# snap-research/3dgp

Measured on AMD Instinct MI355X. Metric: generator-forward img/s @256^2, 64 steps, higher is better.
Workload: dtype f32; 1 GPU; BASELINE configs[2]: ImageNet 256x256, 64(+64) ray steps, cmax 512, c_dim 1000, tri-plane 512^2 x 96, full HIP path; batch_per_gpu=16, global_batch=16, img_resolution=256, num_ray_steps=64, depth_adaptor=False, parallelism=dp1 (batch-sharded, weights replicated)

## Files before the change

### 3dgp_amd/_lib.py

```python
import ctypes
import os
from ctypes import POINTER, c_char_p, c_double, c_float, c_int, c_int32, c_int64, c_void_p

import torch

_HERE = os.path.dirname(os.path.abspath(__file__))
LIB_PATH = os.path.join(_HERE, 'csrc', 'libtdgp_hip.so')

P = c_void_p
_PROTOTYPES = {
    'tdgp_version': (c_int, []),
    'tdgp_last_error': (c_char_p, []),
    'tdgp_profile_enable': (c_int, [c_int]),
    'tdgp_profile_report': (c_int64, [c_char_p, c_int64]),
    'tdgp_device_fault': (c_int, [c_int]),
    'tdgp_bias_act': (c_int, [P, P, P, c_int64, c_int, c_int64, c_int, c_float, c_float, c_float, c_int, P]),
    'tdgp_bias_act_grad': (c_int, [P, P, P, P, P, P, c_int64, c_int, c_int64, c_int, c_int, c_float, c_float, c_float, c_int, P]),
    'tdgp_upfirdn2d': (c_int, [P, P, P, c_int, c_int, c_int, c_int, POINTER(c_int64), c_int, c_int, POINTER(c_int64),
                               c_int, c_int, c_int, c_int, c_int, c_int, c_int, c_int, c_int, c_int, c_int, c_float, c_int, P]),
    'tdgp_modconv_pack_bytes': (c_int64, [c_int, c_int, c_int]),
    'tdgp_modconv_pack': (c_int, [P, P, c_int, c_int, c_int, P]),
    'tdgp_modconv2d_workspace_bytes': (c_int64, [c_int, c_int, c_int, c_int, c_int, c_int, c_int]),
    'tdgp_modconv2d_takes_folded_up2': (c_int, [c_int, c_int, c_int, c_int, c_int]),
    'tdgp_modconv2d_path': (c_int, [c_int, c_int, c_int, c_int, c_int, c_int, c_int, c_int, c_int]),
    'tdgp_conv2d': (c_int, [P, P, P, P, c_int, c_int, c_int, c_int, c_int, c_int, c_int, c_int, c_int, c_int, P]),
    'tdgp_conv2d_weight_grad_workspace_bytes': (c_int64, [c_int, c_int, c_int, c_int, c_int]),
    'tdgp_conv2d_weight_grad': (c_int, [P, P, P, P, c_int64, c_int, c_int, c_int, c_int, c_int, c_int, c_int, c_int, c_int, c_int, P]),
    'tdgp_conv_transpose2d_x2': (c_int, [P, P, P, P, c_int, c_int, c_int, c_int, c_int, P, c_int64, P]),
    'tdgp_set_conv_arith': (c_int, [c_int]),
    'tdgp_modconv_wsq_offset': (c_int64, [c_int, c_int, c_int]),
    'tdgp_demod_batch': (c_int, [P, P, P, c_int, c_int, c_int, P]),
    'tdgp_modconv2d': (c_int, [P, P, P, P, P, c_int64, P, POINTER(c_float), P, P, c_int, c_int, c_int, c_int, c_int, c_int, c_int,
                               c_int, c_int, c_float, c_float, c_float, c_int, c_int, P, c_int64, P]),
    'tdgp_modconv2d_bf16': (c_int, [P, P, P, P, P, c_int64, P, POINTER(c_float), P, P, c_int, c_int, c_int, c_int, c_int, c_int, c_int,
                                    c_int, c_int, c_float, c_float, c_float, c_int, c_int, P, c_int64, P]),
    'tdgp_cast_f32_bf16': (c_int, [P, P, c_int64, P]),
    'tdgp_style_affine': (c_int, [P, P, P, P, P, P, c_int, c_int, c_int, c_int, P]),
    'tdgp_cam2world': (c_int, [P, P, P, P, c_int, P]),
    'tdgp_sample_rays': (c_int, [P, P, c_int, P, P, P, P, c_int, c_int, c_int, P]),
    'tdgp_sample_stratified': (c_int, [P, P, P, c_int64, c_int, c_int, c_float, c_float, P]),
    'tdgp_density_activation': (c_int, [P, P, c_int64, c_int, c_float, P]),
    'tdgp_planes_to_hwc': (c_int, [P, P, c_int, c_int, c_int, c_int, P]),
    'tdgp_triplane_features': (c_int, [P, P, P, c_int, c_int64, c_int, c_int, c_int, c_float, P]),
    'tdgp_triplane_field': (c_int, [P, P, P, P, P, P, P, P, P, P, c_float, P, P, c_int, c_int64, c_int, c_int, c_int, c_int, c_int, c_int, c_float,
                                    c_int, P]),
    'tdgp_ray_march': (c_int, [P, P, P, P, P, P, P, c_int64, c_int, c_int, c_int, c_int, c_float, c_float, P]),
    'tdgp_triplane_field_grad_workspace_bytes': (c_int64, [c_int, c_int64, c_int, c_int]),
    'tdgp_triplane_field_grad': (c_int, [P, P, P, P, P, P, P, P, P, P, P, P, P, P, c_int64, c_int, c_int64, c_int, c_int, c_int, c_int, c_float, c_int, P]),
    'tdgp_triplane_field_deep': (c_int, [P, P, P, P, P, P, P, c_int, P, c_float, P, P, c_int, c_int64, c_int, c_int, c_int, c_int, c_int, c_int, c_float,
                                         c_int, P]),
    'tdgp_triplane_field_deep_grad_workspace_bytes': (c_int64, [c_int, c_int64, c_int, c_int, c_int]),
    'tdgp_triplane_field_deep_grad': (c_int, [P, P, P, P, c_int, P, P, P, P, P, P, c_int64, c_int, c_int64, c_int, c_int, c_int, c_int, c_float, c_int, P]),
    'tdgp_ray_march_grad': (c_int, [P, P, P, P, P, P, P, P, c_int64, c_int, c_int, c_int, c_int, c_float, P]),
    'tdgp_sample_importance': (c_int, [P, P, P, P, P, P, P, P, c_int64, c_int, c_int, c_int, c_int, P]),
    'tdgp_unify_samples': (c_int, [P, P, P, c_int, P, P, P, c_int, P, P, P, P, c_int64, c_int, P]),
    'tdgp_importance_from_coarse': (c_int, [P, P, P, P, P, P, P, c_int64, c_int, c_int, c_int, c_int, c_float, c_float, c_float, c_float, P]),
    'tdgp_merge_composite': (c_int, [P, P, c_int, P, P, c_int, P, P, P, P, P, P, c_int64, c_int, c_int, c_float, c_float, P]),
    'tdgp_render_fused_workspace_bytes': (c_int64, [c_int, c_int64, c_int, c_int]),
    'tdgp_render_fused': (c_int, [P] * 13 + [c_int, c_int64, c_int, c_int, c_int, c_int, c_int, c_int, c_int, c_float, c_float, c_float, c_int, c_int, c_float, P, c_int64, P]),
    'tdgp_rays_to_image': (c_int, [P, P, c_int, c_int, P]),
    'tdgp_frames_to_grid_u8': (c_int, [P, c_int64, c_int, c_int, c_int, P, c_int, c_int, c_int64, c_int64, c_int, c_int, c_int, c_float, c_float, P]),
    'tdgp_ppl_frames': (c_int, [P, c_int64, c_int, c_int, c_int, c_int, c_int, P, P]),
    'tdgp_pair_sqdist_workspace_bytes': (c_int64, [c_int64, c_int64]),
    'tdgp_pair_sqdist': (c_int, [P, c_int64, c_int64, c_double, P, P, c_int64, P]),
    'tdgp_voxel_coords': (c_int, [P, c_int64, c_int64, c_int, c_float, c_float, c_float, c_float, P]),
    'tdgp_mcubes_workspace_bytes': (c_int64, [c_int, c_int, c_int]),
    'tdgp_mcubes_count': (c_int, [P, c_int, c_int, c_int, c_float, P, c_int64, P]),
    'tdgp_mcubes_emit': (c_int, [P, c_int, c_int, c_int, c_float, P, c_int64, P, c_int64, P, c_int64, P]),
    'tdgp_iso_bracket': (c_int, [P, c_int64, P, c_int64, c_int, c_int, c_float, P, P, P]),
    'tdgp_iso_locate': (c_int, [P, c_int64, P, P, P, c_int64, P, P, P, c_int64, c_int, c_int, c_float, c_float, c_float, P, P, P, P]),
    'tdgp_iso_shade': (c_int, [P, P, P, c_int64, c_int, POINTER(c_float), c_float, POINTER(c_float), POINTER(c_float), P, P, P]),
    'tdgp_mesh_visibility': (c_int, [P, c_int64, P, c_int64, P, P, P, c_int, c_int, c_int, c_float, c_int, P, P]),
    'tdgp_mesh_resolve': (c_int, [P, P, c_int64, P, c_int64, P, P, c_int64, c_float, c_float, P, P, P, P, P, P, P, P]),
    'tdgp_mesh_shade': (c_int, [P, P, P, P, c_int64, c_int, POINTER(c_float), c_float, POINTER(c_float), POINTER(c_float), P, P]),
    'tdgp_mesh_visibility_ms': (c_int, [P, c_int64, P, c_int64, P, P, c_int, c_int, c_int, c_int, c_float, c_int, P, P]),
    'tdgp_mesh_resolve_ms': (c_int, [P, P, c_int64, P, c_int64, P, P, c_int, c_int, c_int, c_int, c_float, P, P, P, c_int, c_int, c_int, c_int, c_int, c_int,
                                     POINTER(c_float), c_float, POINTER(c_float), POINTER(c_float), P, P, P, P, P, P, P]),
    'tdgp_mesh_labels_workspace_bytes': (c_int64, [c_int64, c_int64]),
    'tdgp_mesh_labels': (c_int, [P, c_int64, c_int64, P, P, c_int64, P]),
    'tdgp_mesh_component_ids_workspace_bytes': (c_int64, [c_int64]),
    'tdgp_mesh_component_ids': (c_int, [P, c_int64, P, P, c_int64, P]),
    'tdgp_mesh_component_stats': (c_int, [P, P, c_int64, c_int64, P, c_int64, P, P, P, P, P, P, P, P]),
# ... 108 lines not shown

def byte_workspace(query_name, dims, device, refusal, at_least=0):
    need = int(getattr(load(), query_name)(*dims))
    if need < 0:
        raise refusal
    return torch.empty([max(need, at_least)], dtype=torch.uint8, device=device), need


def require_cuda(t, what):
    if not (isinstance(t, torch.Tensor) and t.is_cuda):
        raise RuntimeError(f'{what} must reside on the GPU (got {getattr(t, "device", type(t))}); the HIP ops have no CPU path')


def f32c(t):
    if t.dtype != torch.float32:
        t = t.float()
    return t.contiguous()


def profile_enable(on=True):
    load().tdgp_profile_enable(int(bool(on)))


def profile_report():
    lib = load()
    need = lib.tdgp_profile_report(None, 0)
    buf = ctypes.create_string_buffer(int(need) + 16)
    lib.tdgp_profile_report(buf, len(buf))
    out = {}
    for line in buf.value.decode().splitlines():
        name, n, tot, mn, mx = line.split()
        out[name] = dict(launches=int(n), total_ms=float(tot), avg_ms=float(tot) / max(int(n), 1), min_ms=float(mn), max_ms=float(mx))
    return out


def device_fault(clear=False):
    return int(load().tdgp_device_fault(int(bool(clear))))


def raise_on_device_fault(where=''):
    code = device_fault(clear=True)
    if code:
        raise RuntimeError(f'libtdgp_hip: device fault {code} reported{" in " + where if where else ""}: a bounded in-kernel wait ran out, '
                           'the results of that launch are invalid (the fault word has been cleared)')


def set_conv_arith(mode):
    lib = load()
    prev = int(lib.tdgp_set_conv_arith(int(mode)))
    if prev < 0:
        msg = lib.tdgp_last_error()
        raise RuntimeError(f'tdgp_set_conv_arith failed ({prev}): {msg.decode() if msg else "?"}')
    return prev
```

### 3dgp_amd/build.py

```python
import os
import subprocess
import sys
from concurrent.futures import ThreadPoolExecutor

HERE = os.path.dirname(os.path.abspath(__file__))
CSRC = os.path.join(HERE, 'csrc')
LIB = os.path.join(CSRC, 'libtdgp_hip.so')
SOURCES = ['core.hip', 'bias_act.hip', 'upfirdn2d.hip', 'modconv.hip', 'conv_grad.hip', 'camera_rays.hip', 'frames_grid.hip', 'field.hip', 'field_deep.hip', 'sampling.hip', 'render_grad.hip', 'render_fused.hip', 'geometry.hip', 'iso_surface.hip', 'mesh_raster.hip', 'mesh_components.hip', 'mesh_surface.hip', 'mesh_simplify.hip', 'mesh_texture.hip', 'metrics.hip', 'pair_dist.hip', 'gaussian.hip', 'augment.hip', 'step_tail.hip', 'resample.hip']
HEADERS = ['common.h', 'device_scan.h', 'shade.h', 'mesh_bary.h', 'mesh_hit.h', 'modconv_bf16.inc', 'modconv_wino.inc', 'modconv_wino4.inc', 'modconv_wino4f.inc', 'modconv_host.inc', 'field_body.inc', 'field_grad.inc', 'field_walk2.inc', 'mc_table.inc', os.path.join('..', '..', 'include', 'tdgp.h')]
FLAGS = ['--offload-arch=gfx950', '-O3', '-std=c++17', '-ffp-contract=off', '-fPIC', '-fvisibility=hidden',
         '-Wno-unused-result']


def _hipcc():
    for c in (os.environ.get('HIPCC'), '/opt/rocm/bin/hipcc', 'hipcc'):
        if c and (os.path.isabs(c) and os.path.exists(c) or not os.path.isabs(c)):
            return c
    raise RuntimeError('hipcc not found')


def _stale(target, deps):
    if not os.path.exists(target):
        return True
    t = os.path.getmtime(target)
    return any(os.path.getmtime(d) > t for d in deps)


def _isa_check_module():
    sys.path.insert(0, HERE)
    try:
        import isa_check
    finally:
        sys.path.pop(0)
    return isa_check


def _verify_isa(asm_path, what, check_name):
    isa_check = _isa_check_module()
    skip = os.environ.get('TDGP_SKIP_ISA_CHECK', '0') not in ('', '0')
    try:
        res = getattr(isa_check, check_name)(open(asm_path).read())
        bad = [(k, why, ins) for k, (_, v) in res.items() for why, ins in v]
        msg = None
        if not res:
            msg = f'no {what} instantiation found in the listing'
        elif bad:
            msg = '; '.join(f'{k}: {why} | {ins}' for k, why, ins in bad[:8])
    except isa_check.IsaListingError as e:
        res, msg = {}, f'listing not understood: {e}'
    if msg:
        full = f'ISA check of {what} failed (3dgp_amd/isa_check.py): {msg}'
        if skip:
            import warnings
            warnings.warn(full + ' -- TDGP_SKIP_ISA_CHECK is set: continuing')
            return res
        os.remove(asm_path)
        raise RuntimeError(full + ' (TDGP_SKIP_ISA_CHECK=1 downgrades this to a warning)')
    return res


def verify_field_isa(asm_path):
    return _verify_isa(asm_path, 'triplane_walk2_kernel', 'check_walk2_asm')


def verify_modconv_isa(asm_path):
    res = dict(_verify_isa(asm_path, 'conv3_wino4_kernel', 'check_wino4_asm'))
    res.update(_verify_isa(asm_path, 'conv3_wino4f_kernel', 'check_wino4f_asm'))
    res.update(_verify_isa(asm_path, 'torgb_mfma_kernel (FAST)', 'check_torgb_asm'))
    return res


def build_native(force=False, verbose=False):
    hipcc = _hipcc()
    objdir = os.path.join(CSRC, 'build')
    os.makedirs(objdir, exist_ok=True)
    hdrs = [os.path.join(CSRC, h) for h in HEADERS]
    jobs = []
    for src in SOURCES:
        s = os.path.join(CSRC, src)
        o = os.path.join(objdir, src.replace('.hip', '.o'))
        if force or _stale(o, [s] + hdrs):
            jobs.append((s, o))

    def compile_one(job):
        s, o = job
        cmd = [hipcc] + FLAGS + ['-c', s, '-o', o]
        if verbose:
            print(' '.join(cmd), file=sys.stderr)
        r = subprocess.run(cmd, capture_output=True, text=True)
        if r.returncode != 0:
            raise RuntimeError(f'hipcc failed for {s}:\n{r.stderr}')
        return o

    checked = [('field.hip', 'field.s', verify_field_isa), ('modconv.hip', 'modconv.s', verify_modconv_isa)]
    todo = []
    for src, lst, fn in checked:
        sp, ap = os.path.join(CSRC, src), os.path.join(objdir, lst)
        if any(s == sp for s, _ in jobs) or _stale(ap, [sp] + hdrs):
            todo.append((sp, ap, fn))

    def asm_one(item):
        sp, ap, _ = item
        r = subprocess.run([hipcc] + FLAGS + ['-S', '--cuda-device-only', '-o', ap, sp], capture_output=True, text=True)
        if r.returncode != 0:
            raise RuntimeError(f'hipcc -S failed for {sp}:\n{r.stderr}')

    with ThreadPoolExecutor(max_workers=min(8, max(1, len(jobs) + len(todo)))) as ex:
        futs = [ex.submit(asm_one, it) for it in todo]
        list(ex.map(compile_one, jobs))
        for f in futs:
            f.result()
    for _, ap, fn in todo:
        fn(ap)
    objs = [os.path.join(objdir, s.replace('.hip', '.o')) for s in SOURCES]
    if force or jobs or _stale(LIB, objs):
        cmd = [hipcc, '--offload-arch=gfx950', '-shared', '-fPIC', '-o', LIB] + objs
        r = subprocess.run(cmd, capture_output=True, text=True)
        if r.returncode != 0:
            raise RuntimeError(f'link failed:\n{r.stderr}')
    return LIB


if __name__ == '__main__':
    print(build_native(force='--force' in sys.argv, verbose=True))
```

### 3dgp_amd/csrc/modconv.hip

```cpp
#include <type_traits>
#include "common.h"
#include <stdlib.h>

#define TDGP_WAVE_INDEX(tid) __builtin_amdgcn_readfirstlane((tid) >> 6)

namespace {

typedef float f32x16 __attribute__((ext_vector_type(16)));

constexpr int KC3 = 4;

struct TapTable {
    int ntaps, halo;
    int tap_w[25];
    int tap_off_y[25];
    int tap_off_x[25];
    int gridH, gridW;
};

struct EpiParams {
    const float* __restrict__ dcoef; const float* __restrict__ noise; const float* __restrict__ bias; const float* __restrict__ skip;
    float* __restrict__ y;
    int64_t noise_bstride;
    float fir[16];
// ... 2076 lines not shown
                    float v = acc[o] * d;
                    if (YBF) v = fir_round_bf16(v);
                    if (p.noise && ox0 + lx + o < p.OW) {
                        const float nq[4] = {nzv[hrow].x, nzv[hrow].y, nzv[hrow].z, nzv[hrow].w};
                        v = v + (nz_vec ? nq[o] : p.noise[b * p.noise_bstride + (int64_t)oy * p.OW + ox0 + lx + o]);
                        if (YBF) v = fir_round_bf16(v);
                    }
                    v = v + bv;
                    if constexpr (LRELU) {
                        v = __builtin_fmaxf(v, v * p.alpha) * p.gain;
                        if (p.clamp >= 0.f) v = __builtin_amdgcn_fmed3f(v, -p.clamp, p.clamp);
                    }
                    else {
                        v = act_apply(v, p.act, p.alpha) * p.gain;
                        if (p.clamp >= 0.f) v = v < -p.clamp ? -p.clamp : (v > p.clamp ? p.clamp : v);
                    }
                    out[o] = v;
                }
                if constexpr (YBF) {
                    uint16_t* yp = p.y16 + yoff;
                    if (ox0 + lx + 3 < p.OW && (p.OW & 3) == 0) *(uint2*)yp = make_uint2(fir_pack_bf16(out[0], out[1]), fir_pack_bf16(out[2], out[3]));
                    else
                        for (int o = 0; o < 4 && ox0 + lx + o < p.OW; o++) yp[o] = (uint16_t)(fir_pack_bf16(out[o], 0.f) & 0xffffu);
                } else {
                    float* yp = p.y + yoff;
                    if (ox0 + lx + 3 < p.OW && (p.OW & 3) == 0) *(float4*)yp = make_float4(out[0], out[1], out[2], out[3]);
                    else
                        for (int o = 0; o < 4 && ox0 + lx + o < p.OW; o++) yp[o] = out[o];
                }
            }
        }
    }
}

__global__ __launch_bounds__(256) void z_gather_kernel(const float* __restrict__ z, float* __restrict__ y, int64_t rows, int OHt, int OWt, int P2, int GS2,
                                                       int ksplit, int64_t zslice) {
    for (int64_t r = blockIdx.x; r < rows; r += gridDim.x) {
        const int i = (int)(r % OHt);
        const int64_t bc = r / OHt;
        const float* zp = z + bc * 2 * GS2 + (i & 1) * GS2 + (int64_t)(i >> 1) * P2;
        float* yp = y + r * OWt;
        for (int j = threadIdx.x; j < OWt; j += blockDim.x) {
            float v = zp[j];
            for (int k = 1; k < ksplit; k++) v += zp[k * zslice + j];
            yp[j] = v;
        }
    }
}

#include "modconv_bf16.inc"
#include "modconv_wino.inc"
#include "modconv_wino4.inc"
#include "modconv_wino4f.inc"

__global__ __launch_bounds__(1024) void demod_kernel(const float* __restrict__ styles, const float* __restrict__ wsq, float* __restrict__ d, int B,
                                                    int Cin, int Cout, int CoutP) {
    __shared__ float red[16][64];
    const int ol = threadIdx.x & 63, cs = threadIdx.x >> 6;
    const int o = blockIdx.x * 64 + ol, b = blockIdx.y;
    float acc = 0.f;
    if (o < Cout)
        for (int c = cs; c < Cin; c += 16) {
            const float s = styles[b * Cin + c];
            acc = fmaf_(s * s, wsq[(int64_t)c * CoutP + o], acc);
        }
    red[cs][ol] = acc;
    __syncthreads();
    if (cs == 0 && o < Cout) {
        float t = 0.f;
#pragma unroll
        for (int k = 0; k < 16; k++) t += red[k][ol];
        d[b * Cout + o] = 1.0f / sqrtf(t + 1e-8f);
    }
}

__global__ __launch_bounds__(1024) void demod_batch_kernel(const float* __restrict__ styles_all, const int64_t* __restrict__ meta, float* __restrict__ dcoef_all, int B) {
    __shared__ float red[16][64];
    const int64_t* m = meta + (int64_t)blockIdx.z * 6;
    const float* wsq = (const float*)m[0];
    const int Cin = (int)m[2], Cout = (int)m[3], CoutP = (int)m[4];
    const float* styles = styles_all + m[1];
    float* d = dcoef_all + m[5];
    const int ol = threadIdx.x & 63, cs = threadIdx.x >> 6;
    const int o = blockIdx.x * 64 + ol, b = blockIdx.y;
    if (blockIdx.x * 64 >= Cout) return;
    float acc = 0.f;
    if (o < Cout)
        for (int c = cs; c < Cin; c += 16) {
            const float s = styles[b * Cin + c];
            acc = fmaf_(s * s, wsq[(int64_t)c * CoutP + o], acc);
        }
    red[cs][ol] = acc;
    __syncthreads();
    if (cs == 0 && o < Cout) {
        float t = 0.f;
#pragma unroll
        for (int k = 0; k < 16; k++) t += red[k][ol];
        d[b * Cout + o] = 1.0f / sqrtf(t + 1e-8f);
    }
}

__global__ __launch_bounds__(256) void pack_kernel(const float* __restrict__ w, float* __restrict__ wp, float* __restrict__ wsq, int Cout, int Cin, int T,
                                                  int KC, int CoutP, int nchunks) {
    const int64_t total = (int64_t)nchunks * T * KC * CoutP;
    for (int64_t i = blockIdx.x * (int64_t)blockDim.x + threadIdx.x; i < total; i += (int64_t)gridDim.x * blockDim.x) {
        const int c8 = (int)(i % KC);
// ... 37 lines not shown
```

### 3dgp_amd/csrc/modconv_host.inc

```

constexpr int W4_VCAP_MB = 4095;
constexpr int W4_VSMALL_MB = 192;
constexpr int W4_VSMALL_MINB = 2;
constexpr int WINO_MIN_CIN = 64;

namespace {

inline int round_up(int a, int b) { return (a + b - 1) / b * b; }

struct PackInfo {
    int T, KC, CoutP, nchunks, niter16, nch32, nch8, nch4, nsl64;
    int64_t wp_floats, wsq_floats, wsplit_floats, wbf_floats, wino_floats, wino4_floats;
    int64_t wp, wsq, wsplit, wbf, wino, wino4, total;
};
inline PackInfo pack_info(int Cout, int Cin, int k) {
    PackInfo pi;
    pi.T = k * k;
    pi.KC = KC3;
    pi.CoutP = round_up(Cout, 4);
    pi.nchunks = round_up((Cin + pi.KC - 1) / pi.KC, k == 1 ? 16 : 2);
    pi.wp_floats = (int64_t)pi.nchunks * pi.T * pi.KC * pi.CoutP;
    pi.wsq_floats = (int64_t)Cin * pi.CoutP;
    pi.niter16 = (Cin + 15) / 16;
    pi.wsplit_floats = k == 3 ? (int64_t)pi.niter16 * 9 * 3 * pi.CoutP * 8 : 0;
// ... 41 lines not shown
    p.ksplit = ks;
    p.partial = partial;
    dim3 grid(gx, gy, ks);
    TDGP_LAUNCH("conv_mfma_kernel", (conv_mfma_kernel<MTW, NTW, WM, WN, KCS, MAXT>), grid, dim3(256), lds, s, p);
    if (ks > 1)
        TDGP_LAUNCH("splitk_reduce_kernel", splitk_reduce_kernel, dim3((int)min((int64_t)2048, cdiv64(slice, 256))), dim3(256), 0, s, partial, ks, p.e);
    return 0;
}

inline int tail_ksplit(int blocks, int niter, double flop, int64_t slice_floats, int max_ks) {
    double best = 1e30;
    int ks = 1;
    for (int k = 1; k <= max_ks && k <= 4 && niter / k >= 16; k++) {
        const int n = blocks * k, full = n / 512, rem = n % 512;
        const double rounds = full + (rem == 0 ? 0.0 : (rem <= 256 ? 0.7 : 1.0));
        const double t = rounds * (flop / n) / (100e12 / 512) * 1e6 + (k - 1) * (double)slice_floats * 4.0 / 4e12 * 1e6;
        if (t < best * 0.97) { best = t; ks = k; }
    }
    return ks;
}

struct UpPlan { int cfg, BM, BN, G1, GS, ksplit; int64_t zslice; };
inline UpPlan up_plan(int B, int Cin, int Cout, int H, int W) {
    UpPlan u;
    u.cfg = Cout > 64 ? 0 : 1;
    u.BM = Cout > 64 ? 128 : 64; u.BN = Cout > 64 ? 64 : 128;
    u.G1 = W + 2;
    u.GS = round_up((H + 1) * (W + 2), 32);
    u.zslice = (int64_t)B * Cout * 4 * u.GS;
    const int blocks = cdiv(B * u.GS, u.BN) * cdiv(Cout, u.BM);
    const int niter = cdiv(Cin, 4);
    int ks;
    if (blocks < 256) {
        ks = pick_ksplit(blocks, niter);
        const int64_t cap = ((int64_t)64 << 20) / 4;
        while (ks > 1 && ks * u.zslice > cap) ks--;
    } else {
        ks = tail_ksplit(blocks, niter, 2.0 * Cin * Cout * 9.0 * H * W * B, u.zslice, 4);
    }
    u.ksplit = ks;
    return u;
}

template <int MTW, int NTW, int WM, int WN, bool DEEP>
void launch_upconv(const UpParams& u, hipStream_t s) {
    constexpr int BM = 32 * MTW * WM, BN = 32 * NTW * WN, NW = WM * WN;
    constexpr int stage = 2 * (9 * BM * 4 + 2 * (BN + 2) * 4), epi = NW * 32 * UP_CT_W;
    const size_t lds = (size_t)(stage > epi ? stage : epi) * sizeof(float);
    TDGP_ONCE_PER_DEVICE((void)hipFuncSetAttribute((const void*)upconv_mfma_kernel<MTW, NTW, WM, WN, DEEP>, hipFuncAttributeMaxDynamicSharedMemorySize, (int)lds););
    dim3 grid(cdiv(u.B * u.GS, BN), cdiv(u.Cout, BM), u.ksplit);
    TDGP_LAUNCH("upconv_mfma_kernel", (upconv_mfma_kernel<MTW, NTW, WM, WN, DEEP>), grid, dim3(64 * NW), lds, s, u);
}

template <int MT, bool RESIDENT, bool FAST, bool XBF>
void launch_torgb_v(const RgbParams& r, hipStream_t s) {
    constexpr int BM = 32 * MT;
    const size_t lds = (size_t)(16 * BM * 4 + 16 * 128 * 4 + BM) * sizeof(float);
    TDGP_ONCE_PER_DEVICE((void)hipFuncSetAttribute((const void*)torgb_mfma_kernel<MT, RESIDENT, FAST, XBF>, hipFuncAttributeMaxDynamicSharedMemorySize, (int)lds););
    RgbParams rr = r;
    const int64_t ntiles = cdiv64(r.P, 128);
    if constexpr (RESIDENT && FAST && !XBF) {
        const int cus = tdgp_cu_count();
        if (r.e.skip && ntiles >= (int64_t)cus * 8) {
            constexpr size_t lds_ws = (size_t)(16 * BM * 4 + 2 * 16 * 128 * 4 + 4 * MT * 32 * CT_LD + BM) * sizeof(float);
            TDGP_ONCE_PER_DEVICE((void)hipFuncSetAttribute((const void*)torgb_ws_kernel<MT>, hipFuncAttributeMaxDynamicSharedMemorySize, (int)lds_ws););
            const int64_t blocks = (int64_t)cus * 4;
            rr.tpb = (int)cdiv64(ntiles, blocks);
            TDGP_LAUNCH("torgb_mfma_kernel", (torgb_ws_kernel<MT>), dim3((unsigned)cdiv64(ntiles, rr.tpb)), dim3(512), lds_ws, s, rr);
            return;
        }
    }
    rr.tpb = RESIDENT ? (int)max((int64_t)1, min((int64_t)8, ntiles / 2048)) : 1;
    TDGP_LAUNCH("torgb_mfma_kernel", (torgb_mfma_kernel<MT, RESIDENT, FAST, XBF>), dim3((unsigned)cdiv64(ntiles, rr.tpb)), dim3(256), lds, s, rr);
}

template <int MT, bool XBF = false>
void launch_torgb(const RgbParams& r, hipStream_t s) {
    const bool fast = r.lw >= 0 && r.e.clamp < 0.f && r.e.gain == 1.f;
    if constexpr (XBF) {
        if (r.Cin <= 64) launch_torgb_v<MT, true, false, true>(r, s); else launch_torgb_v<MT, false, false, true>(r, s);
    } else {
        if (r.Cin <= 64) { if (fast) launch_torgb_v<MT, true, true, false>(r, s); else launch_torgb_v<MT, true, false, false>(r, s); }
        else { if (fast) launch_torgb_v<MT, false, true, false>(r, s); else launch_torgb_v<MT, false, false, false>(r, s); }
    }
}

template <int KS, int MTW, int NTW, int WM, int WN>
int launch_conv3(Conv3Params& p, float* partial, int64_t partial_floats, hipStream_t s) {
    constexpr int BM = 32 * MTW * WM, NT = NTW * WN, R = KS / 2;
    constexpr int stage = 2 * (KS * KS * BM * 4 + (NT + 2 * R) * (32 + 2 * R) * 4) + 5 * BM, epi = 4 * 32 * CT_LD;
    const size_t lds = (size_t)(stage > epi ? stage : epi) * sizeof(float);
    TDGP_ONCE_PER_DEVICE((void)hipFuncSetAttribute((const void*)conv3_mfma_kernel<KS, MTW, NTW, WM, WN>, hipFuncAttributeMaxDynamicSharedMemorySize, (int)lds););
    const int gx = (p.W >> 5) * cdiv(p.B * (p.H + R), NT), gy = cdiv(p.Cout, BM);
    const int niter = cdiv(p.Cin, 4);
    const int64_t slice = (int64_t)p.B * p.Cout * p.H * p.W;
    const int max_ks = (int)min((int64_t)32, partial_floats / slice);
    int ks = gx * gy < 256 ? pick_ksplit(gx * gy, niter) : tail_ksplit(gx * gy, niter, 2.0 * p.Cin * p.Cout * KS * KS * p.H * p.W * p.B, 2 * slice, max_ks);
    if (ks > max_ks) ks = max_ks;
    if (ks < 1) ks = 1;
    p.ksplit = ks;
    p.partial = partial;
    TDGP_LAUNCH("conv_mfma_kernel", (conv3_mfma_kernel<KS, MTW, NTW, WM, WN>), dim3(gx, gy, ks), dim3(256), lds, s, p);
    if (ks > 1)
        TDGP_LAUNCH("splitk_reduce_kernel", splitk_reduce_kernel, dim3((int)min((int64_t)2048, cdiv64(slice, 256))), dim3(256), 0, s, partial, ks, p.e);
    return 0;
}

inline int pick_tw_log2(int gridW) {
    int tw = 4, lg = 2;
    while (tw < 32 && tw < gridW) { tw <<= 1; lg++; }
    return lg;
}

// ... 370 lines not shown
        const size_t lds = (size_t)(2 * 3 * 3 * 64 * 32 + 3 * 2 * 130 * 32 + (2 * 8 * 256 + 8 * 64) * 4 + 2 * 64 * 4);
        TDGP_ONCE_PER_DEVICE((void)hipFuncSetAttribute((const void*)upconv3s_mfma_kernel, hipFuncAttributeMaxDynamicSharedMemorySize, (int)lds););
        TDGP_LAUNCH("upconv_mfma_kernel", upconv3s_mfma_kernel, dim3(cdiv(B * pl.GS, 128), cdiv(Cout, 64)), dim3(256), lds, L.s, q);
    } else {
        const UpParams u = make_up(B, Cin, Cout, H, W, L.pi, pl, L.x, L.wp, L.styles, z);
        if (pl.cfg == 0) launch_upconv<2, 1, 2, 2, true>(u, L.s);
        else launch_upconv<2, 1, 1, 4, false>(u, L.s);
    }
    launch_fir(make_fir(L.e, z, pl, H, W, L.plan.up_split ? 1 : pl.ksplit, false), L.plan.fir_tile, false, L.s);
}

inline ConvCall query_call(int B, int Cin, int Cout, int H, int W, int k, int up, int out_layout, int flags) {
    const bool lrelu = (flags & TDGP_PATHQ_LRELU) != 0, aligned = (flags & TDGP_PATHQ_ALIGNED) != 0;
    return ConvCall{B, Cin, Cout, H, W, k, up, out_layout, out_layout == 1 ? 4 : 0,
                    (flags & TDGP_PATHQ_STYLES) != 0, (flags & TDGP_PATHQ_SKIP) != 0, (flags & TDGP_PATHQ_NOISE) != 0, (flags & TDGP_PATHQ_DEMODULATE) != 0,
                    lrelu ? 3 : 1, lrelu ? 0.2f : 0.f, lrelu ? 1.41421356f : 1.f, -1.f, aligned, aligned, g_conv_arith};
}

}

TDGP_API int64_t tdgp_modconv_pack_bytes(int Cout, int Cin, int k) {
    if (Cout < 1 || Cin < 1 || (k != 1 && k != 3 && k != 5)) return -1;
    return pack_info(Cout, Cin, k).total * (int64_t)sizeof(float);
}

TDGP_API int tdgp_modconv_pack(const float* weight, void* wpack, int Cout, int Cin, int k, tdgp_stream_t stream) {
    TDGP_CHECK(weight && wpack, TDGP_EINVAL, "modconv_pack: null pointer");
    TDGP_CHECK(Cout >= 1 && Cin >= 1, TDGP_EINVAL, "modconv_pack: bad channel counts");
    TDGP_CHECK(k == 1 || k == 3 || k == 5, TDGP_EUNSUPPORTED, "modconv_pack: kernel size %d not on the generator path (1, 3 or 5)", k);
    const PackInfo pi = pack_info(Cout, Cin, k);
    float* wp = (float*)wpack;
    TDGP_LAUNCH("pack_kernel", pack_kernel, dim3((int)min((int64_t)4096, cdiv64(pi.wp_floats, 256))), dim3(256), 0, (hipStream_t)stream, weight, wp + pi.wp,
                       wp + pi.wsq, Cout, Cin, pi.T, pi.KC, pi.CoutP, pi.nchunks);
    if (pi.wsplit_floats > 0)
        TDGP_LAUNCH("pack_kernel", pack_split_kernel, dim3((int)min((int64_t)4096, cdiv64(pi.wsplit_floats, 256))), dim3(256), 0, (hipStream_t)stream, weight,
                    (uint32_t*)(wp + pi.wsplit), Cout, Cin, pi.CoutP, pi.niter16);
    if (pi.wbf_floats > 0)
        TDGP_LAUNCH("pack_kernel", pack_bf16_kernel, dim3((int)min((int64_t)4096, cdiv64(pi.wbf_floats, 256))), dim3(256), 0, (hipStream_t)stream, weight,
                    (uint32_t*)(wp + pi.wbf), Cout, Cin, pi.CoutP, pi.nch32);
    if (pi.wino_floats > 0)
        TDGP_LAUNCH("pack_kernel", pack_wino_kernel, dim3((int)min((int64_t)4096, cdiv64(pi.wino_floats, 256))), dim3(256), 0, (hipStream_t)stream, weight,
                    wp + pi.wino, Cout, Cin, pi.CoutP, pi.nch8);
    if (pi.wino4_floats > 0)
        TDGP_LAUNCH("pack_kernel", pack_wino4_kernel, dim3((int)min((int64_t)4096, cdiv64(pi.wino4_floats, 256))), dim3(256), 0, (hipStream_t)stream, weight,
                    wp + pi.wino4, Cout, Cin, cdiv(Cout, W4_BM), pi.nch4);
    TDGP_LAUNCH_CHECK();
    return TDGP_OK;
}

TDGP_API int tdgp_set_conv_arith(int mode) {
    TDGP_CHECK(mode >= 0 && mode <= 4, TDGP_EINVAL, "set_conv_arith: mode %d (0 = fp32 MFMA, Winograd F(4x4,3x3) / F(2x2,3x3) where they pay; 1 = split-bf16 MFMA with fp32 accumulation; 2 = fp32 MFMA, direct sums only; 3 = as 0 without F(4x4); 4 = as 0 with the F(4x4) input transform always as a pass of its own)", mode);
    const int old = g_conv_arith;
    g_conv_arith = mode;
    return old;
}

TDGP_API int tdgp_modconv2d_takes_folded_up2(int B, int Cin, int Cout4, int H, int W) {
    return (B >= 1 && (Cout4 & 3) == 0 && plan_modconv(query_call(B, Cin, Cout4, H, W, 3, 1, 2, TDGP_PATHQ_ALIGNED)).path == TDGP_PATH_WINO4_FOLDED) ? 1 : 0;
}

TDGP_API int tdgp_modconv2d_path(int B, int Cin, int Cout, int H, int W, int k, int up, int out_layout, int flags) {
    TDGP_CHECK(B >= 1 && Cin >= 1 && Cout >= 1 && H >= 1 && W >= 1, TDGP_EINVAL, "modconv2d_path: bad shape");
    TDGP_CHECK(k == 1 || k == 3 || k == 5, TDGP_EUNSUPPORTED, "modconv2d_path: kernel size %d not supported (1, 3 or 5)", k);
    TDGP_CHECK(up == 1 || (up == 2 && k == 3), TDGP_EUNSUPPORTED, "modconv2d_path: up=%d with k=%d not supported", up, k);
    const ConvCall c = query_call(B, Cin, Cout, H, W, k, up, out_layout, flags);
    TDGP_CHECK(!c.has_skip || (up == 1 && k == 1 && (H % 2) == 0 && (W % 2) == 0), TDGP_EINVAL, "modconv2d_path: skip needs k=1, up=1 and even H/W");
    TDGP_CHECK(!c.demodulate || c.has_styles, TDGP_EINVAL, "modconv2d_path: demodulate needs styles");
    TDGP_CHECK(out_layout == 0 || (out_layout == 2 && k == 3 && up == 1 && (Cout & 3) == 0 && !c.has_skip) || (out_layout == 1 && up == 1 && k == 1), TDGP_EINVAL,
               "modconv2d_path: out_layout %d does not go with k=%d, up=%d", out_layout, k, up);
    TDGP_CHECK((int64_t)B * Cin * H * W < ((int64_t)1 << 30) && (int64_t)B * Cout * (H * up + 1) * (W * up + 1) <= INT32_MAX, TDGP_EINVAL,
               "modconv2d_path: tensor too large (activations are addressed through 4 GiB buffer descriptors)");
    TDGP_CHECK(out_layout != 2 || wino4_takes(c), TDGP_EUNSUPPORTED, "modconv2d_path: out_layout 2 is written by the Winograd F(4x4) kernels only");
    return plan_modconv(c).path;
}

TDGP_API int64_t tdgp_modconv2d_workspace_bytes(int B, int Cin, int Cout, int H, int W, int k, int up) {
    return ws_layout(B, Cin, Cout, H, W, k, up).total;
}

TDGP_API int tdgp_modconv2d(const float* x, const void* wpack, const float* styles, const float* dcoef_in, const float* noise, int64_t noise_bstride,
                            const float* bias, const float* fir4x4, const float* skip, float* y, int B, int Cin, int Cout, int H, int W,
                            int k, int up, int demodulate, int act, float alpha, float gain, float clamp, int out_layout, int out_feat,
                            void* workspace, int64_t workspace_bytes, tdgp_stream_t stream) {
    TDGP_CHECK(x && wpack && y, TDGP_EINVAL, "modconv2d: null pointer");
    TDGP_CHECK(B >= 1 && Cin >= 1 && Cout >= 1 && H >= 1 && W >= 1, TDGP_EINVAL, "modconv2d: bad shape");
    TDGP_CHECK(k == 1 || k == 3 || k == 5, TDGP_EUNSUPPORTED, "modconv2d: kernel size %d not supported (1, 3 or 5)", k);
    TDGP_CHECK(up == 1 || (up == 2 && k == 3), TDGP_EUNSUPPORTED, "modconv2d: up=%d with k=%d not supported", up, k);
    TDGP_CHECK(up == 1 || fir4x4, TDGP_EINVAL, "modconv2d: up=2 needs the 4x4 resample filter");
    TDGP_CHECK(!skip || (up == 1 && k == 1 && fir4x4 && (H % 2) == 0 && (W % 2) == 0), TDGP_EINVAL, "modconv2d: skip needs k=1, up=1, even H/W and the filter");
    TDGP_CHECK(!demodulate || styles, TDGP_EINVAL, "modconv2d: demodulate needs styles");
    TDGP_CHECK(act >= 1 && act <= 9, TDGP_EUNSUPPORTED, "modconv2d: unknown activation %d", act);
    TDGP_CHECK(out_layout == 0 || out_layout == 2 || (out_layout == 1 && out_feat >= 4 && (out_feat % 4) == 0 && (Cout % out_feat) == 0 && up == 1 && k == 1), TDGP_EINVAL,
               "modconv2d: the channel-last plane layout is a ToRGB (k=1, up=1) output");
    TDGP_CHECK(out_layout != 2 || (k == 3 && up == 1 && (Cout & 3) == 0 && !skip && (!demodulate || dcoef_in)), TDGP_EINVAL,
               "modconv2d: out_layout 2 (folded x2 layer) needs k=3, up=1, Cout %% 4 == 0, no skip and precomputed demodulation coefficients");
    const ConvCall c{B, Cin, Cout, H, W, k, up, out_layout, out_feat, styles != nullptr, skip != nullptr, noise != nullptr, demodulate != 0, act, alpha, gain, clamp,
                     io_aligned(x, y, noise, noise_bstride, 16), io_aligned(x, y, noise, noise_bstride, 8), g_conv_arith};
    TDGP_CHECK(out_layout != 2 || wino4_takes(c), TDGP_EUNSUPPORTED,
               "modconv2d: out_layout 2 is written by the Winograd F(4x4) kernels only (shape %dx%d, %d -> %d channels, batch %d does not take them)", H, W, Cin, Cout, B);
    TDGP_CHECK((int64_t)B * Cin * H * W < ((int64_t)1 << 30) && (int64_t)B * Cout * (H * up + 1) * (W * up + 1) <= INT32_MAX, TDGP_EINVAL,
               "modconv2d: tensor too large (activations are addressed through 4 GiB buffer descriptors)");
    ConvLaunch L;
    L.c = c; L.plan = plan_modconv(c); L.pi = pack_info(Cout, Cin, k); L.wl = ws_layout(B, Cin, Cout, H, W, k, up);
    TDGP_CHECK(workspace && workspace_bytes >= L.wl.total, TDGP_EWORKSPACE, "modconv2d: workspace %lld < %lld bytes", (long long)workspace_bytes,
               (long long)L.wl.total);
    L.x = x; L.wp = (const float*)wpack; L.styles = styles; L.ws = (char*)workspace; L.s = (hipStream_t)stream;
// ... 146 lines not shown
```

### 3dgp_amd/isa_check.py

```python
import re


class IsaListingError(RuntimeError):
    """The assembly listing does not have the shape the checker parses (not a violation of the property it checks)."""


def _regs(tok):
    out = set()
    for m in re.finditer(r'v\[(\d+):(\d+)\]', tok):
        out.update(range(int(m.group(1)), int(m.group(2)) + 1))
    for m in re.finditer(r'(?<![\w\[:])v(\d+)\b', tok):
        out.add(int(m.group(1)))
    return out


def _code(lines):
    return [ln for ln in lines if ln.strip() and not ln.strip().startswith(';') and not ln.startswith('.')]


def check_kernel(body, fq):
    heads = [i for i, ln in enumerate(body) if 'Loop Header: Depth=1' in ln]
    if not heads:
        raise IsaListingError("no 'Loop Header: Depth=1' comment in the listing of triplane_walk2_kernel: this hipcc does not annotate loops "
                              '(asm-verbose off, or a different compiler) -- the check cannot locate the producer loop')
# ... 273 lines not shown
    bounds = [0] + [n + 1 for n in ends]
    stages = len(ends)
    for st in range(stages):
        nb = bounds[st + 1] - bounds[st]
        w, ld_ = hw[bounds[st]:bounds[st + 1]], hl[4 * bounds[st]:4 * bounds[st + 1]]
        counts = [int(re.search(r'\((\d+)\)', code[k]).group(1)) for k in w]
        ahead = counts[0] // 4
        want = [4 * min(ahead, nb - 1 - bi) for bi in range(nb)]
        if counts != want or counts[0] % 4 or not (1 <= ahead <= 5 or (ahead == 0 and nb == 1)):
            bad.append((f'wait counts of a stage must be 4 x min(look-ahead, batches left): {want}', str(counts)))
            continue
        if not (ld_[0] < w[0] and all(ld_[4 * (bi + ahead)] > w[bi - 1] for bi in range(1, nb - ahead)) and ld_[-1] < w[nb - ahead - 1 if nb > ahead else 0] + 10 ** 9):
            bad.append(('tap loads and waits of a stage are not interleaved as issued', ''))
        seg = [(k, c) for k, c in enumerate(code[ld_[0]:w[-1] + 1], ld_[0]) if re.match(r'^(buffer_|global_|flat_|scratch_)', c)]
        other = [c for k, c in seg if not (hand[k] and c.startswith('global_load_dwordx4')) and not c.startswith('global_store_dwordx4')]
        if other:
            bad.append(('a vector-memory instruction of the compiler\'s between the hand-counted waits of a stage (the hardware counts it, the hand does not)', other[0]))
        for bi in range(nb - 1):
            st_ = [c for c in code[w[bi]:w[bi + 1]] if c.startswith('global_store_dwordx4')]
            if len(st_) != 1:
                bad.append((f'{len(st_)} stores between two hand-counted waits (one per batch)', ''))
                break
        for n, k in enumerate(ld_):
            m = re.match(r'^global_load_dwordx4 v\[(\d+):(\d+)\]', code[k])
            if not m:
                bad.append(('a hand-issued tap load the checker cannot read', code[k]))
                break
            regs = set(range(int(m.group(1)), int(m.group(2)) + 1))
            hit = None
            for c in code[k + 1:w[n // 4]]:
                ops = c.split(None, 1)[1] if ' ' in c else ''
                used = set()
                for tok in re.findall(r'v\[(\d+):(\d+)\]|\bv(\d+)\b', ops):
                    used |= set(range(int(tok[0]), int(tok[1]) + 1)) if tok[0] else {int(tok[2])}
                if used & regs:
                    hit = c
                    break
            if hit:
                bad.append((f'registers of a tap load in flight are touched before its wait ({code[k].split(",")[0]})', hit))
                break
    return dict(batches=len(hw), tap_loads=len(hl), hand_waits=len(hw), stages=stages), bad


def check_torgb_asm(asm_text):
    lines = asm_text.splitlines()
    out = {}
    for i, ln in enumerate(lines):
        m = re.match(r'^(_ZN\S*torgb_mfma_kernelILi(\d)ELb[01]ELb1ELb0E\S*):', ln) or re.match(r'^(_ZN\S*torgb_ws_kernelILi(\d)E\S*):', ln)
        if not m:
            continue
        end = next((j for j in range(i, len(lines)) if lines[j].strip().startswith('.amdhsa_kernel')), len(lines))
        out[m.group(1)] = check_torgb_kernel(lines[i:end], int(m.group(2)))
    return out
```

### include/tdgp.h

```cpp
#ifndef TDGP_H
#define TDGP_H

#include <stdint.h>

#ifdef __cplusplus
extern "C" {
#endif

#define TDGP_OK            0
#define TDGP_EINVAL       -1
#define TDGP_EUNSUPPORTED -2
#define TDGP_ELAUNCH      -3
#define TDGP_EWORKSPACE   -4

#define TDGP_F32  0
#define TDGP_F16  1
#define TDGP_BF16 2
#define TDGP_F64  3

typedef void* tdgp_stream_t;

int         tdgp_version(void);
const char* tdgp_last_error(void);

// ... 2 lines not shown

int     tdgp_device_fault(int clear);

int tdgp_bias_act(const void* x, const void* b, void* y, int64_t n, int sizeB, int64_t stepB,
                  int act, float alpha, float gain, float clamp, int dtype, tdgp_stream_t stream);

int tdgp_bias_act_grad(const void* x, const void* b, const void* xref, const void* yref, const void* dy, void* y, int64_t n,
                       int sizeB, int64_t stepB, int grad, int act, float alpha, float gain, float clamp, int dtype,
                       tdgp_stream_t stream);

int tdgp_upfirdn2d(const void* x, const float* f, void* y, int N, int C, int inH, int inW,
                   const int64_t* x_strides, int outH, int outW, const int64_t* y_strides,
                   int fH, int fW, int upx, int upy, int downx, int downy,
                   int padx0, int padx1, int pady0, int pady1, int flip, float gain,
                   int dtype, tdgp_stream_t stream);

int64_t tdgp_modconv_pack_bytes(int Cout, int Cin, int k);
int     tdgp_modconv_pack(const float* weight, void* wpack, int Cout, int Cin, int k, tdgp_stream_t stream);
int64_t tdgp_modconv2d_workspace_bytes(int B, int Cin, int Cout, int H, int W, int k, int up);
int     tdgp_modconv2d_takes_folded_up2(int B, int Cin, int Cout4, int H, int W);
typedef enum tdgp_conv_path {
    TDGP_PATH_DIRECT = 0,
    TDGP_PATH_CONV3 = 1,
    TDGP_PATH_SPLIT3 = 2,
    TDGP_PATH_WINO2 = 3,
    TDGP_PATH_WINO4 = 4,
    TDGP_PATH_WINO4F = 5,
    TDGP_PATH_WINO4_SPLITK = 6,
    TDGP_PATH_WINO4_FOLDED = 7,
    TDGP_PATH_UP = 8,
    TDGP_PATH_TORGB = 9,
    TDGP_PATH_CONV1 = 10
} tdgp_conv_path;
enum { TDGP_PATHQ_STYLES = 1, TDGP_PATHQ_SKIP = 2, TDGP_PATHQ_NOISE = 4, TDGP_PATHQ_DEMODULATE = 8, TDGP_PATHQ_ALIGNED = 16, TDGP_PATHQ_LRELU = 32 };
int     tdgp_modconv2d_path(int B, int Cin, int Cout, int H, int W, int k, int up, int out_layout, int flags);
int     tdgp_modconv2d(const float* x, const void* wpack, const float* styles, const float* dcoef, const float* noise,
                       int64_t noise_bstride, const float* bias, const float* fir4x4, const float* skip,
                       float* y, int B, int Cin, int Cout, int H, int W, int k, int up, int demodulate,
                       int act, float alpha, float gain, float clamp, int out_layout, int out_feat,
                       void* workspace, int64_t workspace_bytes, tdgp_stream_t stream);

int     tdgp_modconv2d_bf16(const void* x_bf16, const void* wpack, const float* styles, const float* dcoef, const float* noise,
                            int64_t noise_bstride, const float* bias, const float* fir4x4, const float* skip,
                            void* y, int B, int Cin, int Cout, int H, int W, int k, int up, int demodulate,
                            int act, float alpha, float gain, float clamp, int out_layout, int out_feat,
                            void* workspace, int64_t workspace_bytes, tdgp_stream_t stream);
int     tdgp_cast_f32_bf16(const float* x, void* y_bf16, int64_t n, tdgp_stream_t stream);

int     tdgp_conv_transpose2d_x2(const float* x, const void* wpack, const float* styles, float* y, int B, int Cin, int Cout,
                                 int H, int W, void* workspace, int64_t workspace_bytes, tdgp_stream_t stream);

int     tdgp_set_conv_arith(int mode);

int64_t tdgp_modconv_wsq_offset(int Cout, int Cin, int k);
int     tdgp_demod_batch(const float* styles_all, const int64_t* meta, float* dcoef_all, int B, int num_layers,
                         int max_cout, tdgp_stream_t stream);

int tdgp_style_affine(const float* ws, const float* A, const float* abias, const int32_t* row_meta,
                      const float* row_scale, float* styles, int B, int num_ws, int w_dim, int rows_total,
                      tdgp_stream_t stream);

int64_t tdgp_conv2d_weight_grad_workspace_bytes(int B, int Cin, int Cout, int OH, int k);
int     tdgp_conv2d(const float* x, const float* w, const float* bias, float* y, int B, int Cin, int Cout, int H, int W,
                    int OH, int OW, int k, int stride, int pad, tdgp_stream_t stream);
int     tdgp_conv2d_weight_grad(const float* x, const float* dy, float* dw, void* workspace, int64_t workspace_bytes, int B,
                                int Cin, int Cout, int H, int W, int OH, int OW, int k, int stride, int pad,
                                tdgp_stream_t stream);

int tdgp_cam2world(const float* angles, const float* radius, const float* look_at, float* c2w, int B,
                   tdgp_stream_t stream);
int tdgp_sample_rays(const float* c2w, const float* fov, int fov_stride, const float* patch_scales,
                     const float* patch_offsets, float* ray_o, float* ray_d, int B, int h, int w,
                     tdgp_stream_t stream);


int tdgp_sample_stratified(const float* u, float* sdist, float* tdist, int64_t rays, int S, int marcher,
                           float t_near, float t_far, tdgp_stream_t stream);

int tdgp_density_activation(const float* sigma, float* out, int64_t n, int flags, float density_bias, tdgp_stream_t stream);

int tdgp_planes_to_hwc(const float* planes_nchw, float* planes_hwc, int B, int F, int H, int W,
                       tdgp_stream_t stream);

int tdgp_triplane_features(const float* planes_hwc, const float* coords, float* feats, int B, int64_t P, int F, int H, int W,
                           float scale, tdgp_stream_t stream);

int tdgp_triplane_field(const float* planes_hwc, const float* coords, const float* ray_o, const float* ray_d,
                        const float* t, const float* w0, const float* b0, const float* w1, const float* b1,
                        const float* sigma_noise, float density_noise, float* rgbs, int32_t* tap_idx, int B, int64_t P,
                        int S, int ray_w, int F, int H, int W, int hid, float scale, int marcher, tdgp_stream_t stream);

int64_t tdgp_triplane_field_grad_workspace_bytes(int B, int64_t P, int F, int hid);
int     tdgp_triplane_field_grad(const float* planes_hwc, const float* coords, const float* w0, const float* b0,
                                 const float* w1, const float* b1, const float* d_out, float* d_planes_hwc, float* d_w0,
                                 float* d_b0, float* d_w1, float* d_b1, float* d_coords, void* workspace, int64_t workspace_bytes,
                                 int B, int64_t P, int F, int H, int W, int hid, float scale, int marcher, tdgp_stream_t stream);

int tdgp_triplane_field_deep(const float* planes_hwc, const float* coords, const float* ray_o, const float* ray_d,
                             const float* t, const float* const* w, const float* const* b, int n_layers,
                             const float* sigma_noise, float density_noise, float* rgbs, int32_t* tap_idx, int B, int64_t P,
                             int S, int ray_w, int F, int H, int W, int hid, float scale, int marcher, tdgp_stream_t stream);

int64_t tdgp_triplane_field_deep_grad_workspace_bytes(int B, int64_t P, int F, int hid, int n_layers);
int     tdgp_triplane_field_deep_grad(const float* planes_hwc, const float* coords, const float* const* w, const float* const* b,
                                      int n_layers, const float* d_out, float* d_planes_hwc, float* const* d_w, float* const* d_b,
                                      float* d_coords, void* workspace, int64_t workspace_bytes, int B, int64_t P, int F, int H, int W,
// ... 206 lines not shown
```

Before: 751.9 img/s.

## Add register-prefetched 32-channel streaming toRGB MFMA kernel for large skip layers

Adds a new toRGB kernel that streams 32 input channels per stage, prefetching the next stage's weights, activations and styles into registers while MFMAs run on the current stage in LDS. It applies style modulation on the fly and reuses the pipelined skip output epilogue. Automatic dispatch picks it for non-resident FAST fp32 toRGB layers with a skip input when tiles exceed 8 per CU, and a new API can force either path. This trades a larger register footprint and more barriers per channel for less LDS and more occupancy, with the aim of hiding load latency on the big high-resolution toRGB layers.

```diff
diff --git a/3dgp_amd/_lib.py b/3dgp_amd/_lib.py
--- a/3dgp_amd/_lib.py
+++ b/3dgp_amd/_lib.py
@@ -28,6 +28,7 @@
     'tdgp_conv2d_weight_grad': (c_int, [P, P, P, P, c_int64, c_int, c_int, c_int, c_int, c_int, c_int, c_int, c_int, c_int, c_int, P]),
     'tdgp_conv_transpose2d_x2': (c_int, [P, P, P, P, c_int, c_int, c_int, c_int, c_int, P, c_int64, P]),
     'tdgp_set_conv_arith': (c_int, [c_int]),
+    'tdgp_set_torgb_form': (c_int, [c_int]),
     'tdgp_modconv_wsq_offset': (c_int64, [c_int, c_int, c_int]),
     'tdgp_demod_batch': (c_int, [P, P, P, c_int, c_int, c_int, P]),
     'tdgp_modconv2d': (c_int, [P, P, P, P, P, c_int64, P, POINTER(c_float), P, P, c_int, c_int, c_int, c_int, c_int, c_int, c_int,
@@ -242,3 +243,12 @@
         msg = lib.tdgp_last_error()
         raise RuntimeError(f'tdgp_set_conv_arith failed ({prev}): {msg.decode() if msg else "?"}')
     return prev
+
+
+def set_torgb_form(form):
+    lib = load()
+    prev = int(lib.tdgp_set_torgb_form(int(form)))
+    if prev < 0:
+        msg = lib.tdgp_last_error()
+        raise RuntimeError(f'tdgp_set_torgb_form failed ({prev}): {msg.decode() if msg else "?"}')
+    return prev
diff --git a/3dgp_amd/build.py b/3dgp_amd/build.py
--- a/3dgp_amd/build.py
+++ b/3dgp_amd/build.py
@@ -7,7 +7,7 @@
 CSRC = os.path.join(HERE, 'csrc')
 LIB = os.path.join(CSRC, 'libtdgp_hip.so')
 SOURCES = ['core.hip', 'bias_act.hip', 'upfirdn2d.hip', 'modconv.hip', 'conv_grad.hip', 'camera_rays.hip', 'frames_grid.hip', 'field.hip', 'field_deep.hip', 'sampling.hip', 'render_grad.hip', 'render_fused.hip', 'geometry.hip', 'iso_surface.hip', 'mesh_raster.hip', 'mesh_components.hip', 'mesh_surface.hip', 'mesh_simplify.hip', 'mesh_texture.hip', 'metrics.hip', 'pair_dist.hip', 'gaussian.hip', 'augment.hip', 'step_tail.hip', 'resample.hip']
-HEADERS = ['common.h', 'device_scan.h', 'shade.h', 'mesh_bary.h', 'mesh_hit.h', 'modconv_bf16.inc', 'modconv_wino.inc', 'modconv_wino4.inc', 'modconv_wino4f.inc', 'modconv_host.inc', 'field_body.inc', 'field_grad.inc', 'field_walk2.inc', 'mc_table.inc', os.path.join('..', '..', 'include', 'tdgp.h')]
+HEADERS = ['common.h', 'device_scan.h', 'shade.h', 'mesh_bary.h', 'mesh_hit.h', 'modconv_bf16.inc', 'modconv_wino.inc', 'modconv_wino4.inc', 'modconv_wino4f.inc', 'modconv_rgbstream.inc', 'modconv_host.inc', 'field_body.inc', 'field_grad.inc', 'field_walk2.inc', 'mc_table.inc', os.path.join('..', '..', 'include', 'tdgp.h')]
 FLAGS = ['--offload-arch=gfx950', '-O3', '-std=c++17', '-ffp-contract=off', '-fPIC', '-fvisibility=hidden',
          '-Wno-unused-result']
 
@@ -70,6 +70,15 @@
     return res
 
 
+def verify_rgb_stream_isa(asm_path):
+    return _verify_isa(asm_path, 'rgb_stream_kernel', 'check_rgb_stream_asm')
+
+
+def _verify_modconv_listing(asm_path):
+    verify_modconv_isa(asm_path)
+    verify_rgb_stream_isa(asm_path)
+
+
 def build_native(force=False, verbose=False):
     hipcc = _hipcc()
     objdir = os.path.join(CSRC, 'build')
@@ -92,7 +101,7 @@
             raise RuntimeError(f'hipcc failed for {s}:\n{r.stderr}')
         return o
 
-    checked = [('field.hip', 'field.s', verify_field_isa), ('modconv.hip', 'modconv.s', verify_modconv_isa)]
+    checked = [('field.hip', 'field.s', verify_field_isa), ('modconv.hip', 'modconv.s', _verify_modconv_listing)]
     todo = []
     for src, lst, fn in checked:
         sp, ap = os.path.join(CSRC, src), os.path.join(objdir, lst)
diff --git a/3dgp_amd/csrc/modconv.hip b/3dgp_amd/csrc/modconv.hip
--- a/3dgp_amd/csrc/modconv.hip
+++ b/3dgp_amd/csrc/modconv.hip
@@ -2152,6 +2152,7 @@
 #include "modconv_wino.inc"
 #include "modconv_wino4.inc"
 #include "modconv_wino4f.inc"
+#include "modconv_rgbstream.inc"
 
 __global__ __launch_bounds__(1024) void demod_kernel(const float* __restrict__ styles, const float* __restrict__ wsq, float* __restrict__ d, int B,
                                                     int Cin, int Cout, int CoutP) {
diff --git a/3dgp_amd/csrc/modconv_host.inc b/3dgp_amd/csrc/modconv_host.inc
--- a/3dgp_amd/csrc/modconv_host.inc
+++ b/3dgp_amd/csrc/modconv_host.inc
@@ -117,6 +117,22 @@
     TDGP_LAUNCH("upconv_mfma_kernel", (upconv_mfma_kernel<MTW, NTW, WM, WN, DEEP>), grid, dim3(64 * NW), lds, s, u);
 }
 
+int g_torgb_form = 0;
+
+template <int MT, int NBLK, int NSET, bool PRE>
+void launch_rgb_stream_v(const RgbParams& r, hipStream_t s) {
+    constexpr int BM = 32 * MT;
+    const size_t lds = (size_t)(8 * BM * 4 + 8 * 128 * 4 + BM) * sizeof(float);
+    RgbParams rr = r;
+    rr.tpb = 1;
+    TDGP_LAUNCH("torgb_mfma_kernel", (rgb_stream_kernel<MT, NBLK, NSET, PRE>), dim3((unsigned)cdiv64(r.P, 128)), dim3(256), lds, s, rr);
+}
+template <int MT>
+void launch_rgb_stream(const RgbParams& r, hipStream_t s) {
+    if (r.Cin <= 128) launch_rgb_stream_v<MT, 3, 3, true>(r, s);
+    else launch_rgb_stream_v<MT, 4, 2, false>(r, s);
+}
+
 template <int MT, bool RESIDENT, bool FAST, bool XBF>
 void launch_torgb_v(const RgbParams& r, hipStream_t s) {
     constexpr int BM = 32 * MT;
@@ -124,6 +140,12 @@
     TDGP_ONCE_PER_DEVICE((void)hipFuncSetAttribute((const void*)torgb_mfma_kernel<MT, RESIDENT, FAST, XBF>, hipFuncAttributeMaxDynamicSharedMemorySize, (int)lds););
     RgbParams rr = r;
     const int64_t ntiles = cdiv64(r.P, 128);
+    if constexpr (!RESIDENT && FAST && !XBF) {
+        if (r.e.skip && g_torgb_form != 1 && (g_torgb_form == 2 || ntiles >= (int64_t)tdgp_cu_count() * 8)) {
+            launch_rgb_stream<MT>(r, s);
+            return;
+        }
+    }
     if constexpr (RESIDENT && FAST && !XBF) {
         const int cus = tdgp_cu_count();
         if (r.e.skip && ntiles >= (int64_t)cus * 8) {
@@ -600,6 +622,13 @@
     TDGP_CHECK(mode >= 0 && mode <= 4, TDGP_EINVAL, "set_conv_arith: mode %d (0 = fp32 MFMA, Winograd F(4x4,3x3) / F(2x2,3x3) where they pay; 1 = split-bf16 MFMA with fp32 accumulation; 2 = fp32 MFMA, direct sums only; 3 = as 0 without F(4x4); 4 = as 0 with the F(4x4) input transform always as a pass of its own)", mode);
     const int old = g_conv_arith;
     g_conv_arith = mode;
+    return old;
+}
+
+TDGP_API int tdgp_set_torgb_form(int form) {
+    TDGP_CHECK(form >= 0 && form <= 2, TDGP_EINVAL, "set_torgb_form: form %d (0 = automatic; 1 = 64-channel stages only; 2 = 32-channel stages wherever the shape allows them)", form);
+    const int old = g_torgb_form;
+    g_torgb_form = form;
     return old;
 }
 
diff --git a/3dgp_amd/csrc/modconv_rgbstream.inc b/3dgp_amd/csrc/modconv_rgbstream.inc
--- /dev/null
+++ b/3dgp_amd/csrc/modconv_rgbstream.inc
@@ -0,0 +1,108 @@
+template <int MT, int NBLK, int NSET, bool PRE>
+__global__ __launch_bounds__(256, NBLK) void rgb_stream_kernel(RgbParams p) {
+    constexpr int BM = 32 * MT, BN = 128, NCH = 8;
+    constexpr int AS_SZ = NCH * BM * 4, XS_SZ = NCH * BN * 4;
+    static_assert(AS_SZ + XS_SZ >= 4 * 32 * CT_LD, "the parked output tile lies over As and Xs");
+    extern __shared__ __attribute__((aligned(16))) float smem[];
+    float* As = smem;
+    float* Xs = smem + AS_SZ;
+    float* side = smem + AS_SZ + XS_SZ;
+    const int tid = threadIdx.x, l = tid & 63, wv = TDGP_WAVE_INDEX(tid), l32 = l & 31, half = l >> 5;
+    const int64_t ntiles = (p.P + BN - 1) / BN;
+    const int64_t nb_ = gridDim.x;
+    const int64_t t = ((nb_ & 7) == 0 && nb_ >= 64) ? (int64_t)(blockIdx.x & 7) * (nb_ >> 3) + (blockIdx.x >> 3) : (int64_t)blockIdx.x;
+    if (t >= ntiles) return;
+
+    for (int i = tid; i < BM; i += 256) side[i] = (i < p.Cout && p.e.bias) ? p.e.bias[i] : 0.f;
+
+    const int cq = tid >> 5, pq = tid & 31;
+    uint32_t x_vo = kOOB, s_vo = kOOB;
+    {
+        const int64_t pix = t * BN + 4 * pq;
+        if (pix < p.P) {
+            const int b = (int)(pix / p.HW), inner = (int)(pix - (int64_t)b * p.HW);
+            const int sb = b * p.Cin + 4 * cq;
+            s_vo = (uint32_t)sb * 4u;
+            x_vo = (uint32_t)(sb * p.HW + inner) * 4u;
+        }
+    }
+    const uint32_t hw4 = (uint32_t)p.HW * 4u;
+    const bool cin4 = (p.Cin & 3) == 0;
+    const __amdgpu_buffer_rsrc_t rx = make_rsrc(p.x, p.x_bytes), rw = make_rsrc(p.wp, p.wp_bytes), rs = make_rsrc(p.styles ? p.styles : p.x, p.styles ? p.st_bytes : 0);
+
+    constexpr int NA = (NCH * BM + 255) / 256;
+    uint32_t a_vo[NA];
+#pragma unroll
+    for (int i = 0; i < NA; i++) {
+        const int e = tid + i * 256;
+        a_vo[i] = kOOB;
+        if (e < NCH * BM) {
+            const int chunk = e / BM, col = e % BM;
+            if (col < p.CoutP) a_vo[i] = (uint32_t)(chunk * p.CoutP + col) * 16u;
+        }
+    }
+    const uint32_t a_gstride4 = (uint32_t)(NCH * p.CoutP) * 16u;
+
+    f32x16 acc[MT];
+#pragma unroll
+    for (int m = 0; m < MT; m++)
+#pragma unroll
+        for (int r = 0; r < 16; r++) acc[m][r] = 0.f;
+
+    const int niter = (p.Cin + 31) >> 5;
+    float4 a_reg[NA], xr[4], sr;
+    auto load_stage = [&](int it) {
+        const uint32_t a_so = (uint32_t)it * a_gstride4;
+#pragma unroll
+        for (int i = 0; i < NA; i++) a_reg[i] = buf_load4(rw, a_vo[i], a_so);
+        const uint32_t c0 = (uint32_t)it * 32u;
+#pragma unroll
+        for (int j = 0; j < 4; j++) xr[j] = buf_load4(rx, x_vo, (c0 + j) * hw4);
+        if (p.styles) {
+            if (cin4) sr = buf_load4(rs, s_vo, c0 * 4u);
+            else sr = make_float4(buf_load1(rs, s_vo, c0 * 4u), buf_load1(rs, s_vo, c0 * 4u + 4u), buf_load1(rs, s_vo, c0 * 4u + 8u), buf_load1(rs, s_vo, c0 * 4u + 12u));
+        } else {
+            sr = make_float4(1.f, 1.f, 1.f, 1.f);
+        }
+    };
+    auto store_stage = [&]() {
+#pragma unroll
+        for (int i = 0; i < NA; i++)
+            if (tid + i * 256 < NCH * BM) *(float4*)(As + (tid + i * 256) * 4) = a_reg[i];
+        float* d = Xs + ((cq * BN) + pq) * 4;
+        *(float4*)(d + 0 * 128) = make_float4(xr[0].x * sr.x, xr[1].x * sr.y, xr[2].x * sr.z, xr[3].x * sr.w);
+        *(float4*)(d + 1 * 128) = make_float4(xr[0].y * sr.x, xr[1].y * sr.y, xr[2].y * sr.z, xr[3].y * sr.w);
+        *(float4*)(d + 2 * 128) = make_float4(xr[0].z * sr.x, xr[1].z * sr.y, xr[2].z * sr.z, xr[3].z * sr.w);
+        *(float4*)(d + 3 * 128) = make_float4(xr[0].w * sr.x, xr[1].w * sr.y, xr[2].w * sr.z, xr[3].w * sr.w);
+    };
+
+    const float* Al = As + l32 * 4 + 2 * half;
+    const float* Xl = Xs + (wv * 32 + l32) * 4 + 2 * half;
+    float* ct = smem + wv * (32 * CT_LD);
+    load_stage(0);
+    for (int it = 0; it < niter; it++) {
+        __syncthreads();
+        store_stage();
+        __syncthreads();
+        if (it + 1 < niter) load_stage(it + 1);
+        f32x2 fa[2][MT], fb[2];
+        auto load_frag = [&](int buf, int ch) {
+#pragma unroll
+            for (int m = 0; m < MT; m++) fa[buf][m] = *(const f32x2*)(Al + (ch * BM + m * 32) * 4);
+            fb[buf] = *(const f32x2*)(Xl + ch * BN * 4);
+        };
+        load_frag(0, 0);
+#pragma unroll
+        for (int ch = 0; ch < NCH; ch++) {
+            const int cb = ch & 1;
+            if (ch + 1 < NCH) load_frag(cb ^ 1, ch + 1);
+            __builtin_amdgcn_sched_barrier(0);
+#pragma unroll
+            for (int kk = 0; kk < 2; kk++)
+#pragma unroll
+                for (int m = 0; m < MT; m++) acc[m] = __builtin_amdgcn_mfma_f32_32x32x2f32(fa[cb][m][kk], fb[cb][kk], acc[m], 0, 0, 0);
+        }
+    }
+    __syncthreads();
+    rgb_output_skip_pipelined<MT, true, false, NSET, PRE>(p.e, side, ct, acc, t * BN + wv, p.P, p.lw, p.lhw);
+}
diff --git a/3dgp_amd/isa_check.py b/3dgp_amd/isa_check.py
--- a/3dgp_amd/isa_check.py
+++ b/3dgp_amd/isa_check.py
@@ -349,3 +349,15 @@
         end = next((j for j in range(i, len(lines)) if lines[j].strip().startswith('.amdhsa_kernel')), len(lines))
         out[m.group(1)] = check_torgb_kernel(lines[i:end], int(m.group(2)))
     return out
+
+
+def check_rgb_stream_asm(asm_text):
+    lines = asm_text.splitlines()
+    out = {}
+    for i, ln in enumerate(lines):
+        m = re.match(r'^(_ZN\S*rgb_stream_kernelILi(\d)E\S*):', ln)
+        if not m:
+            continue
+        end = next((j for j in range(i, len(lines)) if lines[j].strip().startswith('.amdhsa_kernel')), len(lines))
+        out[m.group(1)] = check_torgb_kernel(lines[i:end], int(m.group(2)))
+    return out
diff --git a/include/tdgp.h b/include/tdgp.h
--- a/include/tdgp.h
+++ b/include/tdgp.h
@@ -78,6 +78,8 @@
 
 int     tdgp_set_conv_arith(int mode);
 
+int     tdgp_set_torgb_form(int form);
+
 int64_t tdgp_modconv_wsq_offset(int Cout, int Cin, int k);
 int     tdgp_demod_batch(const float* styles_all, const int64_t* meta, float* dcoef_all, int B, int num_layers,
                          int max_cout, tdgp_stream_t stream);
```

After: 753.7 img/s (median of 6 runs). No clear change (+0.2%).
